# isl-org/Open3D

Measured on NVIDIA H100. Metric: icp_iters_per_sec_2M_pts, higher is better.
Workload: dtype f32

## Files before the change

### open3d_b200/csrc/icp.cu

```cuda
#include <cfloat>
#include <cstddef>
#include <algorithm>
#include <climits>
#include <cmath>
#include <new>
#include <vector>

#include "comm.h"
#include "common.cuh"
#include "grid.cuh"
#include "reduce.cuh"

namespace o3db {

static constexpr int64_t kMaxCells = int64_t(1) << 26;
static constexpr int kMaxCellsPerAxis = 4096;
static constexpr double kThinFactor = 8;
static constexpr double kDefaultCellScale = 0.5;


__global__ void bbox_kernel(const float* __restrict__ pts, int64_t n, unsigned* __restrict__ bbox ) {
    float mn[3] = {FLT_MAX, FLT_MAX, FLT_MAX}, mx[3] = {-FLT_MAX, -FLT_MAX, -FLT_MAX};
    for (int64_t i = blockIdx.x * (int64_t)blockDim.x + threadIdx.x; i < n;
         i += (int64_t)gridDim.x * blockDim.x) {
// ... 71 lines not shown
    rank[i] = atomicAdd(&count[k], 1u);
}

__global__ void scatter_index_kernel(int64_t n, const unsigned* __restrict__ start, const unsigned* __restrict__ key,
                                     const unsigned* __restrict__ rank, unsigned* __restrict__ idx_sorted) {
    const int64_t i = blockIdx.x * (int64_t)blockDim.x + threadIdx.x;
    if (i < n) idx_sorted[start[key[i]] + rank[i]] = (unsigned)i;
}
static constexpr unsigned kCanonMaxRun = 2048;
__global__ void canonical_rank_kernel(int64_t n, const unsigned* __restrict__ start, const unsigned* __restrict__ key,
                                      const unsigned* __restrict__ idx_sorted, unsigned* __restrict__ rank) {
    const int64_t j = blockIdx.x * (int64_t)blockDim.x + threadIdx.x;
    if (j >= n) return;
    const unsigned i = idx_sorted[j];
    const unsigned k = key[i];
    const unsigned s = start[k], e = start[k + 1];
    if (e - s == 1 || e - s > kCanonMaxRun) return;
    unsigned below = 0;
    for (unsigned q = s; q < e; ++q) below += __ldg(&idx_sorted[q]) < i ? 1u : 0u;
    rank[i] = below;
}
static int canonical_ranks(int64_t n, const unsigned* start, const unsigned* key, unsigned* rank, cudaStream_t st) {
    unsigned* idx_sorted = nullptr;
    O3DB_CUDA_CHECK(cudaMallocAsync(&idx_sorted, n * sizeof(unsigned), st));
    const unsigned nb = (unsigned)ceil_div(n, 256);
    scatter_index_kernel<<<nb, 256, 0, st>>>(n, start, key, rank, idx_sorted);
    O3DB_LAUNCH_CHECK();
    canonical_rank_kernel<<<nb, 256, 0, st>>>(n, start, key, idx_sorted, rank);
    O3DB_LAUNCH_CHECK();
    O3DB_CUDA_CHECK(cudaFreeAsync(idx_sorted, st));
    return O3DB_OK;
}

static constexpr int kSrcChunkBytes = 5 * 32 * 4;
struct SrcBlocked {
    char* base;
    __host__ __device__ static size_t bytes(int64_t n_pad) { return (size_t)(n_pad / 32) * kSrcChunkBytes; }
    __device__ __forceinline__ char* chunk(int i) const { return base + (size_t)(i >> 5) * kSrcChunkBytes; }
    __device__ __forceinline__ float* coord(int axis, int i) const {
        return reinterpret_cast<float*>(chunk(i) + 128 * axis) + (i & 31);
    }
    __device__ __forceinline__ int* seed(int i) const { return reinterpret_cast<int*>(chunk(i) + 384) + (i & 31); }
    __device__ __forceinline__ float* clearance(int i) const { return reinterpret_cast<float*>(chunk(i) + 512) + (i & 31); }
};

__global__ void src_blocked_init_kernel(SrcBlocked sb, int64_t n, int64_t n_pad, bool clear_points) {
    const int64_t i = blockIdx.x * (int64_t)blockDim.x + threadIdx.x;
    if (i >= n_pad) return;
    *sb.seed((int)i) = -1;
    *sb.clearance((int)i) = 0.f;
    if (clear_points && i >= n)
        for (int axis = 0; axis < 3; ++axis) *sb.coord(axis, (int)i) = 0.f;
}

__global__ void scatter_source_kernel(const float* __restrict__ pts, int64_t n, Affine T, const unsigned* __restrict__ start,
                                      const unsigned* __restrict__ key, const unsigned* __restrict__ rank, SrcBlocked sb,
                                      int* __restrict__ src_idx) {
    const int64_t i = blockIdx.x * (int64_t)blockDim.x + threadIdx.x;
    if (i >= n) return;
    float x = pts[3 * i], y = pts[3 * i + 1], z = pts[3 * i + 2];
    apply_transform(T.m, x, y, z);
    const unsigned p = start[key[i]] + rank[i];
    *sb.coord(0, (int)p) = x;
    *sb.coord(1, (int)p) = y;
    *sb.coord(2, (int)p) = z;
    src_idx[p] = (int)i;
}

template <bool TRANSFORM>
__global__ void scatter_kernel(const float* __restrict__ pts, const float* __restrict__ nrm, int64_t n,
                               Affine T, const unsigned* __restrict__ start,
                               const unsigned* __restrict__ key, const unsigned* __restrict__ rank,
                               float4* __restrict__ pts4, float4* __restrict__ nrm4) {
    const int64_t i = blockIdx.x * (int64_t)blockDim.x + threadIdx.x;
    if (i >= n) return;
    float x = pts[3 * i], y = pts[3 * i + 1], z = pts[3 * i + 2];
// ... 567 lines not shown
    p[3 * i + 1] = T.m[4] * x + T.m[5] * y + T.m[6] * z;
    p[3 * i + 2] = T.m[8] * x + T.m[9] * y + T.m[10] * z;
}

__global__ void pack_target_color_kernel(const float4* __restrict__ pts4, const float* __restrict__ col,
                                         const float* __restrict__ grad, int64_t m, float4* __restrict__ tcg) {
    const int64_t j = blockIdx.x * (int64_t)blockDim.x + threadIdx.x;
    if (j >= m) return;
    const int64_t o = 3 * (int64_t)__float_as_int(pts4[j].w);
    tcg[j] = make_float4(grad[o], grad[o + 1], grad[o + 2], color_intensity(col[o], col[o + 1], col[o + 2]));
}

__global__ void pack_source_intensity_kernel(const int* __restrict__ src_idx, const float* __restrict__ col,
                                             int64_t n, float* __restrict__ sint) {
    const int64_t i = blockIdx.x * (int64_t)blockDim.x + threadIdx.x;
    if (i >= n) return;
    const int64_t o = 3 * (int64_t)src_idx[i];
    sint[i] = color_intensity(col[o], col[o + 1], col[o + 2]);
}


struct IcpState {
    double T[16];
    double sums[kSumStride];
    double prev_fitness, prev_rmse, fitness, rmse;
    double count;
    float Uf[16];
    int iter;
    int executed;
    int done;
    int converged;
    int status;
    unsigned ticket;
};

struct IcpArgs {
    Grid g;
    const float4* tgt;
    const float4* nrm;
    const unsigned* cs;
    SrcBlocked src;
    const int* src_idx;
    int64_t n;
    double n_total;
    float rr, thr;
    float r1, r1_accept2;
    Robust rk;
    double* partials;
    IcpState* st;
    double* per_iter;
    int64_t* corr_out;
    double rel_fitness, rel_rmse;
    int max_iteration;
    int fuse_finalize;
    const float4* tcg;
    const float* sint;
    float sqrt_lg, sqrt_lp;
    PeerView peer;
    int use_peer;
};

__device__ void set_identity(double* T, float* Uf) {
    for (int i = 0; i < 16; ++i) {
        const double v = (i % 5 == 0) ? 1.0 : 0.0;
        if (T) T[i] = v;
        if (Uf) Uf[i] = (float)v;
    }
}

static constexpr int kIcpThreads = 768;

__device__ void icp_finalize_iteration(const IcpArgs& a, const double* sums, double* s_scratch) {
    IcpState* st = a.st;
    const int lane = threadIdx.x & 31;
    const double count = sums[28];
    const double fitness = count / a.n_total;
    const double rmse = count > 0 ? sqrt(sums[29] / count) : 0.0;
    if (!(fitness > DBL_MIN)) {
        if (lane == 0) {
            st->fitness = fitness;
            st->rmse = rmse;
            st->count = count;
            set_identity(st->T, st->Uf);
            st->converged = 0;
            st->done = 1;
        }
// ... 55 lines not shown
        st->executed += 1;
        if (st->iter != 0 && fabs(st->prev_fitness - fitness) < a.rel_fitness &&
            fabs(st->prev_rmse - rmse) < a.rel_rmse) {
            st->converged = 1;
            st->done = 1;
        } else {
            st->prev_fitness = fitness;
            st->prev_rmse = rmse;
            st->iter += 1;
            if (st->iter >= a.max_iteration) st->done = 1;
        }
    }
}

__device__ void icp_finalize_evaluate(const IcpArgs& a, const double* sums) {
    IcpState* st = a.st;
    const double count = sums[28];
    st->count = count;
    if (count > 0) {
        st->fitness = count / a.n_total;
        st->rmse = sqrt(sums[29] / count);
    } else {
        st->fitness = 0.0;
        st->rmse = 0.0;
        set_identity(st->T, nullptr);
        st->converged = 0;
    }
    set_identity(nullptr, st->Uf);
}


template <bool L2LOSS, int MODE, bool COLORED>
__device__ __forceinline__ bool icp_process_query(const IcpArgs& a, const float* s_U, int i, float px, float py, float pz,
                                                  int jp, float clear_prev, const float4* seed_ts, const float4* seed_nn,
                                                  const float4* seed_cg, float (&acc)[32]) {
    const float ox = px, oy = py, oz = pz;
    apply_transform(s_U, px, py, pz);
    if (__float_as_uint(px) != __float_as_uint(ox)) *a.src.coord(0, i) = px;
    if (__float_as_uint(py) != __float_as_uint(oy)) *a.src.coord(1, i) = py;
    if (__float_as_uint(pz) != __float_as_uint(oz)) *a.src.coord(2, i) = pz;
    unsigned bj = kNoPoint;
    bool handled = false;
    float clear_new = 0.f;
    float4 ts = make_float4(0.f, 0.f, 0.f, 0.f);
    if (jp >= 0) {
        ts = *seed_ts;
        const float sd = dist2_canonical(ts, px, py, pz);
        const float mx = px - ox, my = py - oy, mz = pz - oz;
        const float m2 = fmaf(mz, mz, fmaf(my, my, mx * mx));
        const float moved = m2 > 0.f ? __fmul_ru(m2 * rsqrtf(m2), 1.00001f) : 0.f;
        const float clear = __fsub_rd(clear_prev, moved);
        const float r1 = sd > 0.f ? __fmul_ru(sd * rsqrtf(sd), 1.00001f) : 0.f;
        if (sd <= a.thr) {
            if (r1 < clear) {
                bj = (unsigned)jp;
                clear_new = clear;
                handled = true;
            } else {
                bj = nn_search_seeded_fast(a.g, a.tgt, a.cs, px, py, pz, a.rr, a.thr, sd, handled, clear_new);
            }
        }
    }
    if (!handled) {
        bj = nn_search_slow(&a.g, a.tgt, a.cs, px, py, pz, a.r1, a.r1_accept2, a.rr, a.thr, jp);
        clear_new = 0.f;
    }
    if ((int)bj != jp) *a.src.seed(i) = (int)bj;
    if (__float_as_uint(clear_new) != __float_as_uint(clear_prev)) *a.src.clearance(i) = clear_new;
    int widx = -1;
    if (bj != kNoPoint) {
        const float4 t = (int)bj == jp ? ts : __ldg(&a.tgt[bj]);
        const float d = dist2_canonical(t, px, py, pz);
        widx = __float_as_int(t.w);
        if (MODE == 0) {
            const float4 nn = (int)bj == jp ? *seed_nn : __ldg(&a.nrm[bj]);
            if (COLORED) {
                const float4 cg = (int)bj == jp ? *seed_cg : __ldg(&a.tcg[bj]);
                const float vs[3] = {px, py, pz}, vt[3] = {t.x, t.y, t.z}, nt[3] = {nn.x, nn.y, nn.z};
                const float dit[3] = {cg.x, cg.y, cg.z};
                accumulate_colored<L2LOSS, 32>(acc, a.rk, vs, vt, nt, __ldg(&a.sint[i]), cg.w, dit, a.sqrt_lg, a.sqrt_lp);
            } else {
                accumulate_p2plane<L2LOSS, 32>(acc, a.rk, px, py, pz, t.x, t.y, t.z, nn.x, nn.y, nn.z);
            }
        } else {
            acc[28] += 1.0f;
        }
        acc[29] += d;
    }
    if (MODE == 1 && a.corr_out) a.corr_out[a.src_idx[i]] = (int64_t)widx;
    return bj != kNoPoint;
}

__device__ __forceinline__ void icp_accumulate_chunk(float (&term)[32], bool matched, double& acc64) {
    if (__any_sync(0xffffffffu, matched)) acc64 += (double)warp_transpose_sum32(term);
}

__device__ __forceinline__ bool peer_all_reduce(const PeerView& pv, double* s_final) {
    const int lane = threadIdx.x & 31;
    unsigned long long seq = 0;
    if (lane == 0) seq = *pv.seq + 1;
    seq = __shfl_sync(0xffffffffu, seq, 0);
    const unsigned tag = (unsigned)seq;
    const size_t par = (size_t)(seq & 1ull) * pv.world;
    if (lane < kNumSums) {
        const unsigned long long bits = (unsigned long long)__double_as_longlong(s_final[lane]);
        const unsigned long long w0 = ((unsigned long long)tag << 32) | (bits & 0xffffffffull);
        const unsigned long long w1 = ((unsigned long long)tag << 32) | (bits >> 32);
        for (int p = 0; p < pv.world; ++p) {
            double* dst = pv.box[p] + (par + pv.rank) * kBoxDoubles + 2 * lane;
            asm volatile("st.volatile.global.v2.u64 [%0], {%1, %2};" ::"l"(dst), "l"(w0), "l"(w1) : "memory");
        }
    }
    double acc = 0.0;
    bool ok = true;
    const long long t0 = global_ns();
    constexpr int kBatch = 8;
    for (int r0 = 0; r0 < pv.world && ok; r0 += kBatch) {
        unsigned long long w0[kBatch], w1[kBatch];
        if (lane < kNumSums) {
            unsigned pending = 0;
#pragma unroll
            for (int u = 0; u < kBatch; ++u)
                if (r0 + u < pv.world) pending |= 1u << u;
            while (pending) {
#pragma unroll
                for (int u = 0; u < kBatch; ++u)
                    if (pending & (1u << u)) {
                        const double* src = pv.box[pv.rank] + (par + r0 + u) * kBoxDoubles + 2 * lane;
                        asm volatile("ld.volatile.global.v2.u64 {%0, %1}, [%2];" : "=l"(w0[u]), "=l"(w1[u]) : "l"(src) : "memory");
                    }
#pragma unroll
                for (int u = 0; u < kBatch; ++u)
                    if ((pending & (1u << u)) && (unsigned)(w0[u] >> 32) == tag && (unsigned)(w1[u] >> 32) == tag) pending &= ~(1u << u);
                if (pending) {
                    if (global_ns() - t0 > 4000000000ll) {
                        ok = false;
                        break;
                    }
                }
            }
            if (ok) {
#pragma unroll
                for (int u = 0; u < kBatch; ++u)
                    if (r0 + u < pv.world) acc += __longlong_as_double((long long)((w1[u] << 32) | (w0[u] & 0xffffffffull)));
            }
        }
        ok = __all_sync(0xffffffffu, ok);
    }
    if (lane < kNumSums) s_final[lane] = acc;
    if (lane == 0) *pv.seq = seq;
    __syncwarp();
    return ok;
}

template <int MODE>
__device__ __forceinline__ void icp_block_epilogue(const IcpArgs& a, double (*s_warp)[kSumStride], double* s_final) {
    if (!block_reduce_to_global<kIcpThreads>(s_warp, a.partials, &a.st->ticket, s_final)) return;
    if (a.fuse_finalize) {
        if (threadIdx.x < 32) {
            if (a.use_peer && !peer_all_reduce(a.peer, s_final)) {
                if (threadIdx.x == 0) {
                    a.st->status = 2;
                    a.st->done = 1;
                }
                return;
            }
            if (MODE == 0) icp_finalize_iteration(a, s_final, &s_warp[0][0]);
            else if (threadIdx.x == 0) icp_finalize_evaluate(a, s_final);
        }
    } else if (threadIdx.x < kNumSums) {
        a.st->sums[threadIdx.x] = s_final[threadIdx.x];
    }
}


template <bool COLORED>
struct __align__(16) IcpStage {
    float px[32];
    float py[32];
    float pz[32];
    int jp[32];
    float d2[32];
    float4 ts[32];
    float4 ns[32];
    float4 cg[COLORED ? 32 : 1];
};

__device__ __forceinline__ void bulk_g2s(void* dst, const void* src, unsigned bytes, unsigned long long* b) {
    asm volatile("cp.async.bulk.shared::cluster.global.mbarrier::complete_tx::bytes [%0], [%1], %2, [%3];" ::"r"(
                         smem_u32(dst)),
                 "l"(src), "r"(bytes), "r"(smem_u32(b))
                 : "memory");
}
__device__ __forceinline__ void cp_async16(void* dst, const void* src) {
    asm volatile("cp.async.ca.shared.global [%0], [%1], 16;" ::"r"(smem_u32(dst)), "l"(src) : "memory");
}
__device__ __forceinline__ void cp_async_commit() { asm volatile("cp.async.commit_group;" ::: "memory"); }
__device__ __forceinline__ void cp_async_wait_all() { asm volatile("cp.async.wait_group 0;" ::: "memory"); }

template <bool COLORED>
struct IcpStagedSmem {
    IcpStage<COLORED> stage[kIcpThreads / 32][2];
};

template <bool L2LOSS, int MODE, bool COLORED = false>
__global__ void __launch_bounds__(kIcpThreads, 1)
icp_iteration_kernel(const __grid_constant__ IcpArgs a) {
    extern __shared__ __align__(16) unsigned char smem_raw[];
    IcpStagedSmem<COLORED>& sm = *reinterpret_cast<IcpStagedSmem<COLORED>*>(smem_raw);
    __shared__ double s_warp[kIcpThreads / 32][kSumStride];
    __shared__ double s_final[kSumStride];
    __shared__ float s_U[16];
    __shared__ int s_done;
    __shared__ __align__(8) unsigned long long s_mbar[kIcpThreads / 32][2];
    const int lane = threadIdx.x & 31, w = threadIdx.x >> 5;
    for (int k = threadIdx.x; k < (kIcpThreads / 32) * kSumStride; k += kIcpThreads) (&s_warp[0][0])[k] = 0.0;
    if (threadIdx.x < 2 * (kIcpThreads / 32)) mbar_init(&s_mbar[0][0] + threadIdx.x, 1);
    asm volatile("fence.mbarrier_init.release.cluster;" ::: "memory");
    pdl_wait();
    pdl_launch_dependents();
    if (threadIdx.x == 0) s_done = *(volatile int*)&a.st->done;
    if (threadIdx.x < 16) s_U[threadIdx.x] = a.st->Uf[threadIdx.x];
    __syncthreads();
    if (MODE == 0 && s_done) return;

    const int n = (int)a.n;
    const int stride = gridDim.x * kIcpThreads;
    const int first = blockIdx.x * kIcpThreads + w * 32;
    constexpr unsigned kBytesA = kSrcChunkBytes;
    static_assert(offsetof(IcpStage<COLORED>, py) == 128 && offsetof(IcpStage<COLORED>, pz) == 256 &&
                  offsetof(IcpStage<COLORED>, jp) == 384 && offsetof(IcpStage<COLORED>, d2) == 512 &&
                  offsetof(IcpStage<COLORED>, ts) == kBytesA, "stage A mirrors a chunk record");
    auto issue_a = [&](int c, int q0) {
        if (lane == 0 && q0 < n) {
            IcpStage<COLORED>& sl = sm.stage[w][c & 1];
            unsigned long long* mb = &s_mbar[w][c & 1];
            mbar_arrive_expect_tx(mb, kBytesA);
            bulk_g2s(sl.px, a.src.chunk(q0), kBytesA, mb);
        }
    };
    auto issue_b = [&](int c, int q0) {
        if (q0 < n) {
            IcpStage<COLORED>& sl = sm.stage[w][c & 1];
            mbar_wait(&s_mbar[w][c & 1], (unsigned)(c >> 1) & 1u);
            const int jp = sl.jp[lane];
            if (jp >= 0) {
                cp_async16(&sl.ts[lane], a.tgt + jp);
                if (MODE == 0) cp_async16(&sl.ns[lane], a.nrm + jp);
                if (MODE == 0 && COLORED) cp_async16(&sl.cg[lane], a.tcg + jp);
            }
        }
        cp_async_commit();
    };

    double acc64 = 0.0;
    issue_a(0, first);
    issue_a(1, first + stride);
    issue_b(0, first);
    int c = 0;
    for (int q0 = first; q0 < n; q0 += stride, ++c) {
        IcpStage<COLORED>& sl = sm.stage[w][c & 1];
        cp_async_wait_all();
        const float px = sl.px[lane], py = sl.py[lane], pz = sl.pz[lane];
        const int jp = sl.jp[lane];
        const float clear_prev = sl.d2[lane];
        __syncwarp();
        issue_a(c + 2, q0 + 2 * stride);
        issue_b(c + 1, q0 + stride);
        const int i = q0 + lane;
        float term[32];
#pragma unroll
        for (int k = 0; k < 32; ++k) term[k] = 0.f;
        bool matched = false;
        if (i < n)
            matched = icp_process_query<L2LOSS, MODE, COLORED>(a, s_U, i, px, py, pz, jp, clear_prev, &sl.ts[lane],
                                                               &sl.ns[lane], &sl.cg[COLORED ? lane : 0], term);
        icp_accumulate_chunk(term, matched, acc64);
    }
    if (lane < kNumSums) s_warp[w][lane] = acc64;
    icp_block_epilogue<MODE>(a, s_warp, s_final);
}

template <int MODE>
__global__ void icp_finalize_kernel(IcpArgs a) {
    __shared__ double s_scratch[64];
    if (MODE == 0) {
        if (a.st->done) return;
        icp_finalize_iteration(a, a.st->sums, s_scratch);
    } else if (threadIdx.x == 0) {
        icp_finalize_evaluate(a, a.st->sums);
    }
}


}

struct o3db_icp {
    o3db_nns nns;
    o3db_icp_options opt{};
    cudaStream_t stream = 0;
    const float* src_user = nullptr;
    int64_t n = 0;
    int64_t n_pad = 0;
    double n_total = 0;
    double init_T[16];
    char* src_blk = nullptr;
    int* src_idx = nullptr;
    unsigned* src_key = nullptr;
    unsigned* src_rank = nullptr;
    unsigned* src_start = nullptr;
    double* partials = nullptr;
    double* per_iter = nullptr;
    IcpState* st = nullptr;
    IcpState* h_st = nullptr;
    o3db_comm* comm = nullptr;
    int grid_blocks = 0;
    int64_t src_keys = 0;
    int launched = 0;
    bool l2loss = true;
    bool colored = false;
    const float* src_colors_user = nullptr;
    float4* tcg4 = nullptr;
    float* sint = nullptr;
    double lambda_geometric = 0.968;
};

namespace o3db {

typedef void (*IcpKernel)(IcpArgs);
static IcpKernel icp_kernel_for(const o3db_icp* c, int mode) {
    if (mode == 1) return icp_iteration_kernel<true, 1, false>;
    if (c->colored) return c->l2loss ? icp_iteration_kernel<true, 0, true> : icp_iteration_kernel<false, 0, true>;
    return c->l2loss ? icp_iteration_kernel<true, 0, false> : icp_iteration_kernel<false, 0, false>;
}

static size_t icp_smem_bytes(const o3db_icp* c, int mode) {
    return (c->colored && mode == 0) ? sizeof(IcpStagedSmem<true>) : sizeof(IcpStagedSmem<false>);
}

static cudaError_t launch_icp(const o3db_icp* c, int mode, cudaStream_t st, const IcpArgs& a) {
    return launch_pdl_ex(icp_kernel_for(c, mode), {(unsigned)c->grid_blocks, kIcpThreads, icp_smem_bytes(c, mode)}, st, a);
}
static IcpArgs make_args(o3db_icp* c) {
    IcpArgs a{};
    a.g = c->nns.g;
    a.tgt = c->nns.pts4;
    a.nrm = c->nns.nrm4;
    a.cs = c->nns.cell_start;
    a.src = SrcBlocked{c->src_blk};
    a.src_idx = c->src_idx;
    a.n = c->n;
    a.n_total = c->n_total;
    const float r = (float)c->opt.max_correspondence_distance;
    a.thr = r * r;
    a.rr = r * (1.0f + 1e-6f);
    a.r1 = fminf(fmaxf(c->nns.g.c, 0.5f * (1.0f + 1e-4f) * r), a.rr);
    a.r1_accept2 = (a.r1 * (1.0f - 1e-4f)) * (a.r1 * (1.0f - 1e-4f));
    a.rk.method = c->opt.kernel.method;
    a.rk.scale = (float)c->opt.kernel.scale;
    a.rk.shape = c->opt.kernel.shape;
    a.partials = c->partials;
    a.st = c->st;
    a.per_iter = c->per_iter;
    a.corr_out = nullptr;
    a.rel_fitness = c->opt.relative_fitness;
    a.rel_rmse = c->opt.relative_rmse;
    a.max_iteration = c->opt.max_iteration;
    const PeerView* pv = o3db_comm_peer_view(c->comm);
    a.use_peer = pv ? 1 : 0;
    if (pv) a.peer = *pv;
    a.fuse_finalize = (c->comm && !pv) ? 0 : 1;
    a.tcg = c->tcg4;
    a.sint = c->sint;
    a.sqrt_lg = (float)sqrt(c->lambda_geometric);
    a.sqrt_lp = (float)sqrt(1.0 - c->lambda_geometric);
    return a;
}

static int icp_init_state(o3db_icp* c, cudaStream_t st) {
    IcpState h{};
    for (int i = 0; i < 16; ++i) {
        h.T[i] = c->init_T[i];
        h.Uf[i] = (i % 5 == 0) ? 1.f : 0.f;
    }
    memcpy(c->h_st, &h, sizeof(h));
    O3DB_CUDA_CHECK(cudaMemcpyAsync(c->st, c->h_st, sizeof(IcpState), cudaMemcpyHostToDevice, st));
    src_blocked_init_kernel<<<(unsigned)ceil_div(c->n_pad, kThreads), kThreads, 0, st>>>(SrcBlocked{c->src_blk}, c->n, c->n_pad,
                                                                                         false);
    O3DB_LAUNCH_CHECK();
    c->launched = 0;
    return O3DB_OK;
}

static int icp_gather_source(o3db_icp* c, cudaStream_t st) {
    Affine T0;
    for (int i = 0; i < 16; ++i) T0.m[i] = (float)c->init_T[i];
    if (c->n == 0) return O3DB_OK;
    scatter_source_kernel<<<(unsigned)ceil_div(c->n, kThreads), kThreads, 0, st>>>(c->src_user, c->n, T0, c->src_start,
                                                                                  c->src_key, c->src_rank, SrcBlocked{c->src_blk},
                                                                                  c->src_idx);
    O3DB_LAUNCH_CHECK();
    return O3DB_OK;
}

}

extern "C" {

int o3db_nns_create(const float* points_dev, int64_t num_points, double radius, void* stream, o3db_nns** out) {
    O3DB_REQUIRE(out != nullptr, "o3db_nns_create: out is null");
    *out = nullptr;
    O3DB_REQUIRE(points_dev != nullptr && num_points > 0, "o3db_nns_create: empty point set");
    O3DB_REQUIRE(num_points < INT_MAX, "o3db_nns_create: too many points");
    O3DB_REQUIRE(radius > 0 && std::isfinite(radius), "o3db_nns_create: radius must be positive");
    o3db_nns* s = new (std::nothrow) o3db_nns();
    O3DB_REQUIRE(s != nullptr, "out of host memory");
    const int rc = nns_build(s, points_dev, nullptr, num_points, radius, 1.0, (cudaStream_t)stream);
    if (rc != O3DB_OK) {
        nns_free(s, (cudaStream_t)stream);
        delete s;
        return rc;
    }
    *out = s;
// ... 416 lines not shown
int o3db_icp_create_colored(const float* source_dev, const float* source_colors_dev, int64_t n,
                            const float* target_dev, const float* target_normals_dev, const float* target_colors_dev,
                            const float* target_color_gradients_dev, int64_t m, const double init_T[16],
                            const o3db_icp_options* options, double lambda_geometric, o3db_comm* comm, void* stream,
                            o3db_icp** out) {
    O3DB_REQUIRE(out != nullptr, "o3db_icp_create_colored: out is null");
    *out = nullptr;
    O3DB_REQUIRE(source_colors_dev != nullptr, "Source pointcloud missing colors attribute.");
    O3DB_REQUIRE(target_colors_dev != nullptr, "Target pointcloud missing colors attribute.");
    O3DB_REQUIRE(target_color_gradients_dev != nullptr,
                 "Target pointcloud missing color_gradients attribute (o3db_estimate_color_gradients).");
    O3DB_REQUIRE(lambda_geometric >= 0.0 && lambda_geometric <= 1.0, "lambda_geometric must be in [0, 1]");
    o3db::ColoredInputs col;
    col.source_colors = source_colors_dev;
    col.target_colors = target_colors_dev;
    col.target_color_gradients = target_color_gradients_dev;
    col.lambda_geometric = lambda_geometric;
    return icp_create_impl(source_dev, n, target_dev, target_normals_dev, m, init_T, options, comm, col, stream, out);
}

int o3db_icp_reset(o3db_icp* c, void* stream) {
    O3DB_REQUIRE(c != nullptr, "o3db_icp_reset: null handle");
    cudaStream_t st = (cudaStream_t)stream;
    int rc = icp_gather_source(c, st);
    if (rc) return rc;
    return icp_init_state(c, st);
}

int o3db_icp_iterate(o3db_icp* c, int iterations, void* stream) {
    O3DB_REQUIRE(c != nullptr, "o3db_icp_iterate: null handle");
    cudaStream_t st = (cudaStream_t)stream;
    const int todo = std::min(iterations, c->opt.max_iteration - c->launched);
    IcpArgs a = make_args(c);
    for (int k = 0; k < todo; ++k) {
        launch_icp(c, 0, st, a);
        O3DB_LAUNCH_CHECK();
        if (!a.fuse_finalize) {
            int rc = o3db_comm_allreduce_f64(c->comm, (double*)((char*)c->st + offsetof(IcpState, sums)), kNumSums, st);
            if (rc) return rc;
            icp_finalize_kernel<0><<<1, 32, 0, st>>>(a);
            O3DB_LAUNCH_CHECK();
        }
        c->launched += 1;
    }
    return O3DB_OK;
}

static int icp_read_state(o3db_icp* c, o3db_icp_result* result, double* per_iteration_host, cudaStream_t st) {
    O3DB_CUDA_CHECK(cudaMemcpyAsync(c->h_st, c->st, sizeof(IcpState), cudaMemcpyDeviceToHost, st));
    O3DB_CUDA_CHECK(cudaStreamSynchronize(st));
    const IcpState& h = *c->h_st;
    memcpy(result->transformation, h.T, sizeof(h.T));
    result->fitness = h.fitness;
    result->inlier_rmse = h.rmse;
    result->converged = h.converged;
    result->num_iterations = h.iter;
    result->num_correspondences = (int64_t)h.count;
    if (h.status == 2) {
        set_last_error("multi-GPU exchange timed out: a peer rank did not publish its sums (in-kernel NVLink exchange)");
        return O3DB_ERR_COMM;
    }
    result->status = h.status ? O3DB_ERR_SINGULAR : O3DB_OK;
    if (per_iteration_host && h.executed > 0) {
        O3DB_CUDA_CHECK(cudaMemcpyAsync(per_iteration_host, c->per_iter, (size_t)h.executed * 2 * sizeof(double),
                                        cudaMemcpyDeviceToHost, st));
        O3DB_CUDA_CHECK(cudaStreamSynchronize(st));
    }
    if (h.status) {
        set_last_error("Singular 6x6 linear system detected, tracking failed.");
        return O3DB_ERR_SINGULAR;
    }
    return O3DB_OK;
}


int o3db_icp_finish(o3db_icp* c, o3db_icp_result* result, int64_t* correspondences_dev, double* per_iteration_host,
                    void* stream) {
    O3DB_REQUIRE(c != nullptr && result != nullptr, "o3db_icp_finish: null argument");
    cudaStream_t st = (cudaStream_t)stream;
    IcpArgs a = make_args(c);
    a.corr_out = correspondences_dev;
    launch_icp(c, 1, st, a);
    O3DB_LAUNCH_CHECK();
    if (!a.fuse_finalize) {
        int rc = o3db_comm_allreduce_f64(c->comm, (double*)((char*)c->st + offsetof(IcpState, sums)), kNumSums, st);
        if (rc) return rc;
        icp_finalize_kernel<1><<<1, 32, 0, st>>>(a);
        O3DB_LAUNCH_CHECK();
    }
    return icp_read_state(c, result, per_iteration_host, st);
}

int o3db_icp_state(o3db_icp* c, o3db_icp_result* result, double* per_iteration_host, void* stream) {
// ... 96 lines not shown
```

### open3d_b200/csrc/common.cuh

```cuda
#pragma once

#include <cuda_runtime.h>
#include <stdint.h>

#include <atomic>
#include <cstdarg>
#include <cstdio>
#include <cstring>

#include "../../include/open3d_b200.h"

namespace o3db {

void set_last_error(const char* fmt, ...);
extern std::atomic<uint64_t> g_launch_count;

inline void count_launch(uint64_t n = 1) { g_launch_count.fetch_add(n, std::memory_order_relaxed); }

#define O3DB_CUDA_CHECK(expr)                                                              \
    do {                                                                                   \
        cudaError_t e__ = (expr);                                                          \
        if (e__ != cudaSuccess) {                                                          \
            ::o3db::set_last_error("%s failed: %s (%s:%d)", #expr, cudaGetErrorString(e__), \
                                   __FILE__, __LINE__);                                    \
// ... 17 lines not shown
        if (!(cond)) {                          \
            ::o3db::set_last_error(__VA_ARGS__); \
            return O3DB_ERR_INVALID;            \
        }                                       \
    } while (0)

inline int num_sms() {
    static int sms = 0;
    if (sms == 0) {
        int dev = 0;
        if (cudaGetDevice(&dev) != cudaSuccess) return 132;
        if (cudaDeviceGetAttribute(&sms, cudaDevAttrMultiProcessorCount, dev) != cudaSuccess || sms <= 0)
            sms = 132;
    }
    return sms;
}

inline int64_t ceil_div(int64_t a, int64_t b) { return (a + b - 1) / b; }

void configure_memory_pool();

void* pinned_acquire(size_t bytes);
void pinned_release(void* p);

#ifdef __CUDACC__
__device__ __forceinline__ void pdl_wait() { asm volatile("griddepcontrol.wait;" ::: "memory"); }
__device__ __forceinline__ void pdl_launch_dependents() { asm volatile("griddepcontrol.launch_dependents;" ::: "memory"); }

struct PdlLaunch {
    dim3 grid;
    unsigned block;
    size_t smem = 0;
    unsigned cluster = 0;
};

template <typename... KArgs, typename... Args>
inline cudaError_t launch_pdl_ex(void (*kernel)(KArgs...), const PdlLaunch& l, cudaStream_t st, Args&&... args) {
    cudaLaunchConfig_t cfg{};
    cfg.gridDim = l.grid;
    cfg.blockDim = dim3(l.block);
    cfg.dynamicSmemBytes = l.smem;
    cfg.stream = st;
    cudaLaunchAttribute attr[2];
    attr[0].id = cudaLaunchAttributeProgrammaticStreamSerialization;
    attr[0].val.programmaticStreamSerializationAllowed = 1;
    attr[1].id = cudaLaunchAttributeClusterDimension;
    attr[1].val.clusterDim.x = l.cluster;
    attr[1].val.clusterDim.y = 1;
    attr[1].val.clusterDim.z = 1;
    cfg.attrs = attr;
    cfg.numAttrs = l.cluster > 0 ? 2 : 1;
    return cudaLaunchKernelEx(&cfg, kernel, static_cast<KArgs>(args)...);
}

__device__ __forceinline__ long long global_ns() {
    long long t;
    asm volatile("mov.u64 %0, %%globaltimer;" : "=l"(t));
    return t;
}

__device__ __forceinline__ unsigned smem_u32(const void* p) { return (unsigned)__cvta_generic_to_shared(p); }
__device__ __forceinline__ void mbar_init(unsigned long long* b, unsigned count) {
    asm volatile("mbarrier.init.shared::cta.b64 [%0], %1;" ::"r"(smem_u32(b)), "r"(count) : "memory");
}
__device__ __forceinline__ void mbar_arrive_expect_tx(unsigned long long* b, unsigned bytes) {
    asm volatile("mbarrier.arrive.expect_tx.shared::cta.b64 _, [%0], %1;" ::"r"(smem_u32(b)), "r"(bytes) : "memory");
}
__device__ __forceinline__ void mbar_wait(unsigned long long* b, unsigned parity) {
    unsigned done;
    do {
        asm volatile(
                "{\n\t.reg .pred p;\n\tmbarrier.try_wait.parity.shared::cta.b64 p, [%1], %2;\n\tselp.u32 %0, 1, 0, p;\n\t}"
                : "=r"(done)
                : "r"(smem_u32(b)), "r"(parity)
                : "memory");
    } while (!done);
}

__device__ __forceinline__ double warp_sum(double v) {
#pragma unroll
    for (int o = 16; o > 0; o >>= 1) v += __shfl_xor_sync(0xffffffffu, v, o);
    return v;
}
__device__ __forceinline__ float warp_sum(float v) {
#pragma unroll
// ... 21 lines not shown
```

Before: 15660.

## Cache seed target point and normal in per-source blocked record

```diff
diff --git a/open3d_b200/csrc/icp.cu b/open3d_b200/csrc/icp.cu
--- a/open3d_b200/csrc/icp.cu
+++ b/open3d_b200/csrc/icp.cu
@@ -127,16 +127,21 @@
     return O3DB_OK;
 }
 
-static constexpr int kSrcChunkBytes = 5 * 32 * 4;
+static constexpr int kSrcPlanes = 11;
+static constexpr int kSrcChunkBytes = kSrcPlanes * 32 * 4;
+static constexpr int kPlaneSeed = 3, kPlaneClear = 4, kPlaneT = 5, kPlaneN = 8;
 struct SrcBlocked {
     char* base;
     __host__ __device__ static size_t bytes(int64_t n_pad) { return (size_t)(n_pad / 32) * kSrcChunkBytes; }
     __device__ __forceinline__ char* chunk(int i) const { return base + (size_t)(i >> 5) * kSrcChunkBytes; }
-    __device__ __forceinline__ float* coord(int axis, int i) const {
-        return reinterpret_cast<float*>(chunk(i) + 128 * axis) + (i & 31);
-    }
-    __device__ __forceinline__ int* seed(int i) const { return reinterpret_cast<int*>(chunk(i) + 384) + (i & 31); }
-    __device__ __forceinline__ float* clearance(int i) const { return reinterpret_cast<float*>(chunk(i) + 512) + (i & 31); }
+    __device__ __forceinline__ float* plane(int p, int i) const {
+        return reinterpret_cast<float*>(chunk(i) + 128 * p) + (i & 31);
+    }
+    __device__ __forceinline__ float* coord(int axis, int i) const { return plane(axis, i); }
+    __device__ __forceinline__ float* seed_point(int axis, int i) const { return plane(kPlaneT + axis, i); }
+    __device__ __forceinline__ float* seed_normal(int axis, int i) const { return plane(kPlaneN + axis, i); }
+    __device__ __forceinline__ int* seed(int i) const { return reinterpret_cast<int*>(plane(kPlaneSeed, i)); }
+    __device__ __forceinline__ float* clearance(int i) const { return plane(kPlaneClear, i); }
 };
 
 __global__ void src_blocked_init_kernel(SrcBlocked sb, int64_t n, int64_t n_pad, bool clear_points) {
@@ -778,6 +783,7 @@
     const float4* nrm;
     const unsigned* cs;
     SrcBlocked src;
+    unsigned record_bytes;
     const int* src_idx;
     int64_t n;
     double n_total;
@@ -911,8 +917,8 @@
 
 template <bool L2LOSS, int MODE, bool COLORED>
 __device__ __forceinline__ bool icp_process_query(const IcpArgs& a, const float* s_U, int i, float px, float py, float pz,
-                                                  int jp, float clear_prev, const float4* seed_ts, const float4* seed_nn,
-                                                  const float4* seed_cg, float (&acc)[32]) {
+                                                  int jp, float clear_prev, const float* rec, const float4* seed_cg,
+                                                  float (&acc)[32]) {
     const float ox = px, oy = py, oz = pz;
     apply_transform(s_U, px, py, pz);
     if (__float_as_uint(px) != __float_as_uint(ox)) *a.src.coord(0, i) = px;
@@ -923,7 +929,7 @@
     float clear_new = 0.f;
     float4 ts = make_float4(0.f, 0.f, 0.f, 0.f);
     if (jp >= 0) {
-        ts = *seed_ts;
+        ts = make_float4(rec[32 * kPlaneT], rec[32 * (kPlaneT + 1)], rec[32 * (kPlaneT + 2)], 0.f);
         const float sd = dist2_canonical(ts, px, py, pz);
         const float mx = px - ox, my = py - oy, mz = pz - oz;
         const float m2 = fmaf(mz, mz, fmaf(my, my, mx * mx));
@@ -948,13 +954,26 @@
     if (__float_as_uint(clear_new) != __float_as_uint(clear_prev)) *a.src.clearance(i) = clear_new;
     int widx = -1;
     if (bj != kNoPoint) {
-        const float4 t = (int)bj == jp ? ts : __ldg(&a.tgt[bj]);
+        const bool kept = (int)bj == jp;
+        float4 t = ts, nn;
+        if (kept) {
+            if (MODE == 0) nn = make_float4(rec[32 * kPlaneN], rec[32 * (kPlaneN + 1)], rec[32 * (kPlaneN + 2)], 0.f);
+            if (MODE == 1 && a.corr_out) widx = __float_as_int(__ldg(&a.tgt[bj].w));
+        } else {
+            t = __ldg(&a.tgt[bj]);
+            nn = __ldg(&a.nrm[bj]);
+            widx = __float_as_int(t.w);
+            *a.src.seed_point(0, i) = t.x;
+            *a.src.seed_point(1, i) = t.y;
+            *a.src.seed_point(2, i) = t.z;
+            *a.src.seed_normal(0, i) = nn.x;
+            *a.src.seed_normal(1, i) = nn.y;
+            *a.src.seed_normal(2, i) = nn.z;
+        }
         const float d = dist2_canonical(t, px, py, pz);
-        widx = __float_as_int(t.w);
         if (MODE == 0) {
-            const float4 nn = (int)bj == jp ? *seed_nn : __ldg(&a.nrm[bj]);
             if (COLORED) {
-                const float4 cg = (int)bj == jp ? *seed_cg : __ldg(&a.tcg[bj]);
+                const float4 cg = kept ? *seed_cg : __ldg(&a.tcg[bj]);
                 const float vs[3] = {px, py, pz}, vt[3] = {t.x, t.y, t.z}, nt[3] = {nn.x, nn.y, nn.z};
                 const float dit[3] = {cg.x, cg.y, cg.z};
                 accumulate_colored<L2LOSS, 32>(acc, a.rk, vs, vt, nt, __ldg(&a.sint[i]), cg.w, dit, a.sqrt_lg, a.sqrt_lp);
@@ -1054,14 +1073,10 @@
 
 
 template <bool COLORED>
+constexpr int kIcpSlots = COLORED ? 3 : 2;
+template <bool COLORED>
 struct __align__(16) IcpStage {
-    float px[32];
-    float py[32];
-    float pz[32];
-    int jp[32];
-    float d2[32];
-    float4 ts[32];
-    float4 ns[32];
+    float rec[kSrcPlanes * 32];
     float4 cg[COLORED ? 32 : 1];
 };
 
@@ -1079,7 +1094,7 @@
 
 template <bool COLORED>
 struct IcpStagedSmem {
-    IcpStage<COLORED> stage[kIcpThreads / 32][2];
+    IcpStage<COLORED> stage[kIcpThreads / 32][kIcpSlots<COLORED>];
 };
 
 template <bool L2LOSS, int MODE, bool COLORED = false>
@@ -1091,10 +1106,10 @@
     __shared__ double s_final[kSumStride];
     __shared__ float s_U[16];
     __shared__ int s_done;
-    __shared__ __align__(8) unsigned long long s_mbar[kIcpThreads / 32][2];
+    __shared__ __align__(8) unsigned long long s_mbar[kIcpThreads / 32][kIcpSlots<COLORED>];
     const int lane = threadIdx.x & 31, w = threadIdx.x >> 5;
     for (int k = threadIdx.x; k < (kIcpThreads / 32) * kSumStride; k += kIcpThreads) (&s_warp[0][0])[k] = 0.0;
-    if (threadIdx.x < 2 * (kIcpThreads / 32)) mbar_init(&s_mbar[0][0] + threadIdx.x, 1);
+    if (threadIdx.x < kIcpSlots<COLORED> * (kIcpThreads / 32)) mbar_init(&s_mbar[0][0] + threadIdx.x, 1);
     asm volatile("fence.mbarrier_init.release.cluster;" ::: "memory");
     pdl_wait();
     pdl_launch_dependents();
@@ -1106,54 +1121,56 @@
     const int n = (int)a.n;
     const int stride = gridDim.x * kIcpThreads;
     const int first = blockIdx.x * kIcpThreads + w * 32;
-    constexpr unsigned kBytesA = kSrcChunkBytes;
-    static_assert(offsetof(IcpStage<COLORED>, py) == 128 && offsetof(IcpStage<COLORED>, pz) == 256 &&
-                  offsetof(IcpStage<COLORED>, jp) == 384 && offsetof(IcpStage<COLORED>, d2) == 512 &&
-                  offsetof(IcpStage<COLORED>, ts) == kBytesA, "stage A mirrors a chunk record");
-    auto issue_a = [&](int c, int q0) {
+    static_assert(offsetof(IcpStage<COLORED>, cg) == kSrcChunkBytes, "a slot's record mirrors a chunk record");
+    const unsigned record_bytes = a.record_bytes;
+    auto chunk_start = [&](unsigned c) { return (int64_t)first + (int64_t)c * stride; };
+    auto slot = [&](unsigned c) -> IcpStage<COLORED>& { return sm.stage[w][c % kIcpSlots<COLORED>]; };
+    auto issue_record = [&](unsigned c) {
+        const int64_t q0 = chunk_start(c);
         if (lane == 0 && q0 < n) {
-            IcpStage<COLORED>& sl = sm.stage[w][c & 1];
-            unsigned long long* mb = &s_mbar[w][c & 1];
-            mbar_arrive_expect_tx(mb, kBytesA);
-            bulk_g2s(sl.px, a.src.chunk(q0), kBytesA, mb);
+            unsigned long long* mb = &s_mbar[w][c % kIcpSlots<COLORED>];
+            mbar_arrive_expect_tx(mb, record_bytes);
+            bulk_g2s(slot(c).rec, a.src.chunk((int)q0), record_bytes, mb);
         }
     };
-    auto issue_b = [&](int c, int q0) {
-        if (q0 < n) {
-            IcpStage<COLORED>& sl = sm.stage[w][c & 1];
-            mbar_wait(&s_mbar[w][c & 1], (unsigned)(c >> 1) & 1u);
-            const int jp = sl.jp[lane];
-            if (jp >= 0) {
-                cp_async16(&sl.ts[lane], a.tgt + jp);
-                if (MODE == 0) cp_async16(&sl.ns[lane], a.nrm + jp);
-                if (MODE == 0 && COLORED) cp_async16(&sl.cg[lane], a.tcg + jp);
-            }
+    auto wait_record = [&](unsigned c) {
+        mbar_wait(&s_mbar[w][c % kIcpSlots<COLORED>], (c / kIcpSlots<COLORED>) & 1u);
+    };
+    auto issue_colour = [&](unsigned c) {
+        if (chunk_start(c) < n) {
+            IcpStage<COLORED>& sl = slot(c);
+            wait_record(c);
+            const int jp = __float_as_int(sl.rec[32 * kPlaneSeed + lane]);
+            if (jp >= 0) cp_async16(&sl.cg[lane], a.tcg + jp);
         }
         cp_async_commit();
     };
 
     double acc64 = 0.0;
-    issue_a(0, first);
-    issue_a(1, first + stride);
-    issue_b(0, first);
-    int c = 0;
+    for (unsigned c = 0; c + 1 < kIcpSlots<COLORED>; ++c) issue_record(c);
+    if (COLORED) issue_colour(0);
+    unsigned c = 0;
     for (int q0 = first; q0 < n; q0 += stride, ++c) {
-        IcpStage<COLORED>& sl = sm.stage[w][c & 1];
-        cp_async_wait_all();
-        const float px = sl.px[lane], py = sl.py[lane], pz = sl.pz[lane];
-        const int jp = sl.jp[lane];
-        const float clear_prev = sl.d2[lane];
         __syncwarp();
-        issue_a(c + 2, q0 + 2 * stride);
-        issue_b(c + 1, q0 + stride);
+        issue_record(c + kIcpSlots<COLORED> - 1);
+        if (COLORED) {
+            cp_async_wait_all();
+            issue_colour(c + 1);
+        } else {
+            wait_record(c);
+        }
+        const float* rec = &slot(c).rec[lane];
+        const float px = rec[0], py = rec[32], pz = rec[64];
+        const int jp = __float_as_int(rec[32 * kPlaneSeed]);
+        const float clear_prev = rec[32 * kPlaneClear];
         const int i = q0 + lane;
         float term[32];
 #pragma unroll
         for (int k = 0; k < 32; ++k) term[k] = 0.f;
         bool matched = false;
         if (i < n)
-            matched = icp_process_query<L2LOSS, MODE, COLORED>(a, s_U, i, px, py, pz, jp, clear_prev, &sl.ts[lane],
-                                                               &sl.ns[lane], &sl.cg[COLORED ? lane : 0], term);
+            matched = icp_process_query<L2LOSS, MODE, COLORED>(a, s_U, i, px, py, pz, jp, clear_prev, rec,
+                                                               &slot(c).cg[COLORED ? lane : 0], term);
         icp_accumulate_chunk(term, matched, acc64);
     }
     if (lane < kNumSums) s_warp[w][lane] = acc64;
@@ -1196,6 +1213,7 @@
     int grid_blocks = 0;
     int64_t src_keys = 0;
     int launched = 0;
+    bool seeded = false;
     bool l2loss = true;
     bool colored = false;
     const float* src_colors_user = nullptr;
@@ -1217,7 +1235,14 @@
     return (c->colored && mode == 0) ? sizeof(IcpStagedSmem<true>) : sizeof(IcpStagedSmem<false>);
 }
 
-static cudaError_t launch_icp(const o3db_icp* c, int mode, cudaStream_t st, const IcpArgs& a) {
+static unsigned icp_record_bytes(const o3db_icp* c, int mode) {
+    const int planes = !c->seeded ? kPlaneT : (mode == 1 ? kPlaneN : kSrcPlanes);
+    return (unsigned)planes * 32 * 4;
+}
+
+static cudaError_t launch_icp(o3db_icp* c, int mode, cudaStream_t st, IcpArgs a) {
+    a.record_bytes = icp_record_bytes(c, mode);
+    c->seeded = true;
     return launch_pdl_ex(icp_kernel_for(c, mode), {(unsigned)c->grid_blocks, kIcpThreads, icp_smem_bytes(c, mode)}, st, a);
 }
 static IcpArgs make_args(o3db_icp* c) {
@@ -1268,6 +1293,7 @@
                                                                                          false);
     O3DB_LAUNCH_CHECK();
     c->launched = 0;
+    c->seeded = false;
     return O3DB_OK;
 }
 
```

After: 16110, median of 6. 2.8% higher.

## Run multiple ICP iterations in one persistent cooperative kernel with grid barrier

Applied to the files above, without the earlier changes.

```diff
diff --git a/open3d_b200/csrc/common.cuh b/open3d_b200/csrc/common.cuh
--- a/open3d_b200/csrc/common.cuh
+++ b/open3d_b200/csrc/common.cuh
@@ -73,6 +73,7 @@
     unsigned block;
     size_t smem = 0;
     unsigned cluster = 0;
+    bool cooperative = false;
 };
 
 template <typename... KArgs, typename... Args>
@@ -82,16 +83,30 @@
     cfg.blockDim = dim3(l.block);
     cfg.dynamicSmemBytes = l.smem;
     cfg.stream = st;
-    cudaLaunchAttribute attr[2];
-    attr[0].id = cudaLaunchAttributeProgrammaticStreamSerialization;
-    attr[0].val.programmaticStreamSerializationAllowed = 1;
-    attr[1].id = cudaLaunchAttributeClusterDimension;
-    attr[1].val.clusterDim.x = l.cluster;
-    attr[1].val.clusterDim.y = 1;
-    attr[1].val.clusterDim.z = 1;
+    cudaLaunchAttribute attr[3];
+    unsigned n = 0;
+    attr[n].id = cudaLaunchAttributeProgrammaticStreamSerialization;
+    attr[n++].val.programmaticStreamSerializationAllowed = 1;
+    if (l.cluster > 0) {
+        attr[n].id = cudaLaunchAttributeClusterDimension;
+        attr[n].val.clusterDim.x = l.cluster;
+        attr[n].val.clusterDim.y = 1;
+        attr[n++].val.clusterDim.z = 1;
+    }
+    if (l.cooperative) {
+        attr[n].id = cudaLaunchAttributeCooperative;
+        attr[n++].val.cooperative = 1;
+    }
     cfg.attrs = attr;
-    cfg.numAttrs = l.cluster > 0 ? 2 : 1;
-    return cudaLaunchKernelEx(&cfg, kernel, static_cast<KArgs>(args)...);
+    cfg.numAttrs = n;
+    cudaError_t e = cudaLaunchKernelEx(&cfg, kernel, static_cast<KArgs>(args)...);
+    if (e != cudaSuccess && l.cooperative) {
+        (void)cudaGetLastError();
+        cfg.attrs = attr + 1;
+        cfg.numAttrs = n - 1;
+        e = cudaLaunchKernelEx(&cfg, kernel, static_cast<KArgs>(args)...);
+    }
+    return e;
 }
 
 __device__ __forceinline__ long long global_ns() {
diff --git a/open3d_b200/csrc/icp.cu b/open3d_b200/csrc/icp.cu
--- a/open3d_b200/csrc/icp.cu
+++ b/open3d_b200/csrc/icp.cu
@@ -770,6 +770,7 @@
     int converged;
     int status;
     unsigned ticket;
+    unsigned generation;
 };
 
 struct IcpArgs {
@@ -790,6 +791,7 @@
     int64_t* corr_out;
     double rel_fitness, rel_rmse;
     int max_iteration;
+    int iterations;
     int fuse_finalize;
     const float4* tcg;
     const float* sint;
@@ -993,7 +995,7 @@
     double acc = 0.0;
     bool ok = true;
     const long long t0 = global_ns();
-    constexpr int kBatch = 8;
+    constexpr int kBatch = 4;
     for (int r0 = 0; r0 < pv.world && ok; r0 += kBatch) {
         unsigned long long w0[kBatch], w1[kBatch];
         if (lane < kNumSums) {
@@ -1033,23 +1035,52 @@
 }
 
 template <int MODE>
-__device__ __forceinline__ void icp_block_epilogue(const IcpArgs& a, double (*s_warp)[kSumStride], double* s_final) {
+__device__ __forceinline__ void icp_block_epilogue(const IcpArgs& a, double (*s_warp)[kSumStride], double* s_final,
+                                                   bool publish) {
     if (!block_reduce_to_global<kIcpThreads>(s_warp, a.partials, &a.st->ticket, s_final)) return;
+    if (threadIdx.x >= 32) return;
     if (a.fuse_finalize) {
-        if (threadIdx.x < 32) {
-            if (a.use_peer && !peer_all_reduce(a.peer, s_final)) {
-                if (threadIdx.x == 0) {
-                    a.st->status = 2;
-                    a.st->done = 1;
-                }
-                return;
+        if (a.use_peer && !peer_all_reduce(a.peer, s_final)) {
+            if (threadIdx.x == 0) {
+                a.st->status = 2;
+                a.st->done = 1;
             }
-            if (MODE == 0) icp_finalize_iteration(a, s_final, &s_warp[0][0]);
-            else if (threadIdx.x == 0) icp_finalize_evaluate(a, s_final);
+        } else if (MODE == 0) {
+            icp_finalize_iteration(a, s_final, &s_warp[0][0]);
+        } else if (threadIdx.x == 0) {
+            icp_finalize_evaluate(a, s_final);
         }
     } else if (threadIdx.x < kNumSums) {
         a.st->sums[threadIdx.x] = s_final[threadIdx.x];
     }
+    if (publish) {
+        __syncwarp();
+        if (threadIdx.x == 0) {
+            __threadfence();
+            asm volatile("red.release.gpu.global.add.u32 [%0], 1;" ::"l"(&a.st->generation) : "memory");
+        }
+    }
+}
+
+__device__ __forceinline__ void icp_grid_wait(const IcpArgs& a, unsigned want, float* s_U, int* s_done) {
+    IcpState* st = a.st;
+    const long long t0 = global_ns();
+    unsigned ns = 16;
+    for (;;) {
+        unsigned g;
+        asm volatile("ld.acquire.gpu.global.u32 %0, [%1];" : "=r"(g) : "l"(&st->generation) : "memory");
+        if ((int)(g - want) >= 0) break;
+        if (global_ns() - t0 > 4000000000ll) {
+            st->status = 3;
+            st->done = 1;
+            break;
+        }
+        __nanosleep(ns);
+        ns = ns < 256 ? 2 * ns : ns;
+    }
+    *s_done = __ldcg(&st->done);
+#pragma unroll
+    for (int k = 0; k < 16; ++k) s_U[k] = __ldcg(&st->Uf[k]);
 }
 
 
@@ -1075,11 +1106,15 @@
     asm volatile("cp.async.ca.shared.global [%0], [%1], 16;" ::"r"(smem_u32(dst)), "l"(src) : "memory");
 }
 __device__ __forceinline__ void cp_async_commit() { asm volatile("cp.async.commit_group;" ::: "memory"); }
-__device__ __forceinline__ void cp_async_wait_all() { asm volatile("cp.async.wait_group 0;" ::: "memory"); }
+template <int PENDING>
+__device__ __forceinline__ void cp_async_wait() { asm volatile("cp.async.wait_group %0;" ::"n"(PENDING) : "memory"); }
+
+static constexpr int kIcpRing = 2;
+static_assert(kIcpRing >= 2, "A must run at least one chunk ahead of B");
 
 template <bool COLORED>
 struct IcpStagedSmem {
-    IcpStage<COLORED> stage[kIcpThreads / 32][2];
+    IcpStage<COLORED> stage[kIcpThreads / 32][kIcpRing];
 };
 
 template <bool L2LOSS, int MODE, bool COLORED = false>
@@ -1091,14 +1126,20 @@
     __shared__ double s_final[kSumStride];
     __shared__ float s_U[16];
     __shared__ int s_done;
-    __shared__ __align__(8) unsigned long long s_mbar[kIcpThreads / 32][2];
+    __shared__ int s_left;
+    __shared__ unsigned s_want;
+    __shared__ __align__(8) unsigned long long s_mbar[kIcpThreads / 32][kIcpRing];
     const int lane = threadIdx.x & 31, w = threadIdx.x >> 5;
     for (int k = threadIdx.x; k < (kIcpThreads / 32) * kSumStride; k += kIcpThreads) (&s_warp[0][0])[k] = 0.0;
-    if (threadIdx.x < 2 * (kIcpThreads / 32)) mbar_init(&s_mbar[0][0] + threadIdx.x, 1);
+    if (threadIdx.x < kIcpRing * (kIcpThreads / 32)) mbar_init(&s_mbar[0][0] + threadIdx.x, 1);
     asm volatile("fence.mbarrier_init.release.cluster;" ::: "memory");
     pdl_wait();
     pdl_launch_dependents();
-    if (threadIdx.x == 0) s_done = *(volatile int*)&a.st->done;
+    if (threadIdx.x == 0) {
+        s_done = *(volatile int*)&a.st->done;
+        s_left = a.iterations - 1;
+        s_want = __ldcg(&a.st->generation) + 1u;
+    }
     if (threadIdx.x < 16) s_U[threadIdx.x] = a.st->Uf[threadIdx.x];
     __syncthreads();
     if (MODE == 0 && s_done) return;
@@ -1110,18 +1151,18 @@
     static_assert(offsetof(IcpStage<COLORED>, py) == 128 && offsetof(IcpStage<COLORED>, pz) == 256 &&
                   offsetof(IcpStage<COLORED>, jp) == 384 && offsetof(IcpStage<COLORED>, d2) == 512 &&
                   offsetof(IcpStage<COLORED>, ts) == kBytesA, "stage A mirrors a chunk record");
-    auto issue_a = [&](int c, int q0) {
+    auto issue_a = [&](unsigned c, int q0) {
         if (lane == 0 && q0 < n) {
-            IcpStage<COLORED>& sl = sm.stage[w][c & 1];
-            unsigned long long* mb = &s_mbar[w][c & 1];
+            IcpStage<COLORED>& sl = sm.stage[w][c % kIcpRing];
+            unsigned long long* mb = &s_mbar[w][c % kIcpRing];
             mbar_arrive_expect_tx(mb, kBytesA);
             bulk_g2s(sl.px, a.src.chunk(q0), kBytesA, mb);
         }
     };
-    auto issue_b = [&](int c, int q0) {
+    auto issue_b = [&](unsigned c, int q0) {
         if (q0 < n) {
-            IcpStage<COLORED>& sl = sm.stage[w][c & 1];
-            mbar_wait(&s_mbar[w][c & 1], (unsigned)(c >> 1) & 1u);
+            IcpStage<COLORED>& sl = sm.stage[w][c % kIcpRing];
+            mbar_wait(&s_mbar[w][c % kIcpRing], (c / kIcpRing) & 1u);
             const int jp = sl.jp[lane];
             if (jp >= 0) {
                 cp_async16(&sl.ts[lane], a.tgt + jp);
@@ -1132,32 +1173,58 @@
         cp_async_commit();
     };
 
-    double acc64 = 0.0;
-    issue_a(0, first);
-    issue_a(1, first + stride);
-    issue_b(0, first);
-    int c = 0;
-    for (int q0 = first; q0 < n; q0 += stride, ++c) {
-        IcpStage<COLORED>& sl = sm.stage[w][c & 1];
-        cp_async_wait_all();
-        const float px = sl.px[lane], py = sl.py[lane], pz = sl.pz[lane];
-        const int jp = sl.jp[lane];
-        const float clear_prev = sl.d2[lane];
-        __syncwarp();
-        issue_a(c + 2, q0 + 2 * stride);
-        issue_b(c + 1, q0 + stride);
-        const int i = q0 + lane;
-        float term[32];
-#pragma unroll
-        for (int k = 0; k < 32; ++k) term[k] = 0.f;
-        bool matched = false;
-        if (i < n)
-            matched = icp_process_query<L2LOSS, MODE, COLORED>(a, s_U, i, px, py, pz, jp, clear_prev, &sl.ts[lane],
-                                                               &sl.ns[lane], &sl.cg[COLORED ? lane : 0], term);
-        icp_accumulate_chunk(term, matched, acc64);
-    }
-    if (lane < kNumSums) s_warp[w][lane] = acc64;
-    icp_block_epilogue<MODE>(a, s_warp, s_final);
+    unsigned c = 0;
+#pragma unroll
+    for (int k = 0; k < kIcpRing; ++k) issue_a(k, first + k * stride);
+#pragma unroll
+    for (int k = 0; k < kIcpRing - 1; ++k) issue_b(k, first + k * stride);
+    for (;;) {
+        double acc64 = 0.0;
+        for (int q0 = first; q0 < n; q0 += stride, ++c) {
+            IcpStage<COLORED>& sl = sm.stage[w][c % kIcpRing];
+            cp_async_wait<kIcpRing - 2>();
+            const float px = sl.px[lane], py = sl.py[lane], pz = sl.pz[lane];
+            const int jp = sl.jp[lane];
+            const float clear_prev = sl.d2[lane];
+            __syncwarp();
+            issue_a(c + kIcpRing, q0 + kIcpRing * stride);
+            issue_b(c + kIcpRing - 1, q0 + (kIcpRing - 1) * stride);
+            const int i = q0 + lane;
+            float term[32];
+#pragma unroll
+            for (int k = 0; k < 32; ++k) term[k] = 0.f;
+            bool matched = false;
+            if (i < n)
+                matched = icp_process_query<L2LOSS, MODE, COLORED>(a, s_U, i, px, py, pz, jp, clear_prev, &sl.ts[lane],
+                                                                   &sl.ns[lane], &sl.cg[COLORED ? lane : 0], term);
+            icp_accumulate_chunk(term, matched, acc64);
+        }
+        if (lane < kNumSums) s_warp[w][lane] = acc64;
+        const bool more = s_left > 0;
+        if (more) {
+            asm volatile("fence.proxy.async.global;" ::: "memory");
+            __syncwarp();
+#pragma unroll
+            for (int k = 0; k < kIcpRing; ++k) issue_a(c + k, first + k * stride);
+        }
+        icp_block_epilogue<MODE>(a, s_warp, s_final, more);
+        if (!more) return;
+#pragma unroll
+        for (int k = 0; k < kIcpRing - 1; ++k) issue_b(c + k, first + k * stride);
+        if (threadIdx.x == 0) {
+            icp_grid_wait(a, s_want, s_U, &s_done);
+            s_want += 1u;
+            s_left -= 1;
+        }
+        __syncthreads();
+        if (s_done) {
+#pragma unroll
+            for (int k = 0; k < kIcpRing; ++k)
+                if (first + k * stride < n) mbar_wait(&s_mbar[w][(c + k) % kIcpRing], ((c + k) / kIcpRing) & 1u);
+            cp_async_wait<0>();
+            return;
+        }
+    }
 }
 
 template <int MODE>
@@ -1218,7 +1285,8 @@
 }
 
 static cudaError_t launch_icp(const o3db_icp* c, int mode, cudaStream_t st, const IcpArgs& a) {
-    return launch_pdl_ex(icp_kernel_for(c, mode), {(unsigned)c->grid_blocks, kIcpThreads, icp_smem_bytes(c, mode)}, st, a);
+    return launch_pdl_ex(icp_kernel_for(c, mode),
+                         {(unsigned)c->grid_blocks, kIcpThreads, icp_smem_bytes(c, mode), 0, a.iterations > 1}, st, a);
 }
 static IcpArgs make_args(o3db_icp* c) {
     IcpArgs a{};
@@ -1245,6 +1313,7 @@
     a.rel_fitness = c->opt.relative_fitness;
     a.rel_rmse = c->opt.relative_rmse;
     a.max_iteration = c->opt.max_iteration;
+    a.iterations = 1;
     const PeerView* pv = o3db_comm_peer_view(c->comm);
     a.use_peer = pv ? 1 : 0;
     if (pv) a.peer = *pv;
@@ -1750,6 +1819,16 @@
     cudaStream_t st = (cudaStream_t)stream;
     const int todo = std::min(iterations, c->opt.max_iteration - c->launched);
     IcpArgs a = make_args(c);
+    if (todo > 1 && a.fuse_finalize) {
+        a.iterations = todo;
+        if (launch_icp(c, 0, st, a) == cudaSuccess) {
+            count_launch();
+            c->launched += todo;
+            return O3DB_OK;
+        }
+        (void)cudaGetLastError();
+        a.iterations = 1;
+    }
     for (int k = 0; k < todo; ++k) {
         launch_icp(c, 0, st, a);
         O3DB_LAUNCH_CHECK();
@@ -1777,6 +1856,10 @@
     if (h.status == 2) {
         set_last_error("multi-GPU exchange timed out: a peer rank did not publish its sums (in-kernel NVLink exchange)");
         return O3DB_ERR_COMM;
+    }
+    if (h.status == 3) {
+        set_last_error("ICP grid barrier timed out: a block of the iteration kernel did not reach the end of an iteration");
+        return O3DB_ERR_CUDA;
     }
     result->status = h.status ? O3DB_ERR_SINGULAR : O3DB_OK;
     if (per_iteration_host && h.executed > 0) {
diff --git a/profiles/icp_loop_times.py b/profiles/icp_loop_times.py
--- /dev/null
+++ b/profiles/icp_loop_times.py
@@ -0,0 +1,86 @@
+import argparse
+import ctypes as C
+import json
+import os
+import subprocess
+import sys
+
+import numpy as np
+import torch
+
+sys.path.insert(0, os.path.dirname(os.path.dirname(os.path.abspath(__file__))))
+from open3d_b200 import _lib as L
+from tests.synth import make_icp_pair
+
+TARGET_POINTS = 2_000_000
+FIRST, REST = 5, 25
+
+
+def card():
+    q = "name,power.limit,clocks.max.sm"
+    out = subprocess.run(["nvidia-smi", "-i", "0", f"--query-gpu={q}", "--format=csv,noheader"], capture_output=True,
+                         text=True, timeout=30).stdout.strip()
+    name, power, clock = [x.strip() for x in out.split(",")]
+    return {"name": name, "power_limit": power, "max_sm_clock": clock}
+
+
+def main():
+    ap = argparse.ArgumentParser()
+    ap.add_argument("--points", type=int, default=TARGET_POINTS, help="source points")
+    ap.add_argument("--reps", type=int, default=5)
+    ap.add_argument("--label", default="")
+    args = ap.parse_args()
+    if not torch.cuda.is_available():
+        raise SystemExit("icp_loop_times.py needs a CUDA device")
+    torch.cuda.set_device(0)
+    stream = int(torch.cuda.current_stream().cuda_stream)
+    src, tgt, nrm, T_gt = make_icp_pair(TARGET_POINTS, seed=2)
+    if args.points < len(src):
+        src = np.ascontiguousarray(src[:args.points])
+    d = [torch.from_numpy(a).cuda() for a in (src, tgt, nrm)]
+    opt = L.IcpOptions()
+    opt.max_correspondence_distance, opt.max_iteration = 0.05, FIRST + REST
+    opt.relative_fitness = opt.relative_rmse = 0.0
+    opt.kernel = L.RobustKernel(0, 1.0, 1.0)
+    h = C.c_void_p()
+    L.check(L.lib.o3db_icp_create(d[0].data_ptr(), len(src), d[1].data_ptr(), d[2].data_ptr(), len(tgt),
+                                  L.dptr(np.eye(4)), C.byref(opt), None, stream, C.byref(h)))
+    flush = torch.empty(256 << 20, dtype=torch.uint8, device="cuda")
+    res = L.IcpResult()
+    times = []
+    launches = 0
+    for rep in range(2 + args.reps):
+        L.check(L.lib.o3db_icp_reset(h, stream))
+        flush.fill_(1)
+        evs = [torch.cuda.Event(enable_timing=True) for _ in range(4)]
+        l0 = L.launch_count()
+        evs[0].record()
+        L.check(L.lib.o3db_icp_iterate(h, FIRST, stream))
+        evs[1].record()
+        L.check(L.lib.o3db_icp_iterate(h, REST, stream))
+        evs[2].record()
+        L.check(L.lib.o3db_icp_finish(h, C.byref(res), None, None, stream))
+        evs[3].record()
+        torch.cuda.synchronize()
+        launches = L.launch_count() - l0
+        if rep >= 2:
+            times.append([1e3 * evs[k].elapsed_time(evs[k + 1]) for k in range(3)])
+    L.lib.o3db_icp_destroy(h)
+    t = np.array(times)
+    med, mn = np.median(t, axis=0), t.min(axis=0)
+    print(json.dumps({
+        "label": args.label, "card": card(), "points": len(src), "target_points": len(tgt), "reps": args.reps,
+        "first5_us_median": round(float(med[0]), 1), "first5_us_min": round(float(mn[0]), 1),
+        "rest25_us_median": round(float(med[1]), 1), "rest25_us_min": round(float(mn[1]), 1),
+        "aligned_iteration_us_median": round(float(med[1]) / REST, 2),
+        "aligned_iteration_us_min": round(float(mn[1]) / REST, 2),
+        "finish_us_median": round(float(med[2]), 1),
+        "registration_ms_median": round(float(np.median(t.sum(axis=1))) / 1e3, 4),
+        "launches_per_registration": int(launches),
+        "fitness": res.fitness, "inlier_rmse": res.inlier_rmse, "num_iterations": res.num_iterations,
+        "transformation_error_vs_ground_truth": float(np.abs(np.array(res.transformation).reshape(4, 4) - T_gt).max()),
+    }), flush=True)
+
+
+if __name__ == "__main__":
+    main()
```

Result: faster. 15730 before, 15980 after (median of 6 runs) (+1.6%).
